# cvjena/semantic-embeddings

Hardware: AMD Instinct MI355X
Metric: retrieval_Mpairs_per_sec (higher is better)
Workload: dtype f32

## Files before the change

### semantic-embeddings_amd/csrc/rank_rows.hip

```cpp
#include "se_common.h"
#include <stdlib.h>
#include <atomic>
#include <type_traits>

namespace se {

constexpr int RK_THREADS = 512;
constexpr int RK_WAVES = RK_THREADS / WAVE;
constexpr int RK_ITEMS = 16;
constexpr int RK_TILE = RK_THREADS * RK_ITEMS;
constexpr int RK_WCHUNK = RK_TILE / RK_WAVES;
constexpr int RK_NB = 256;

struct RankLds {
    uint32_t gbase[4][RK_NB];
    uint32_t wcnt[RK_WAVES][RK_NB];
    uint32_t tile_start[RK_NB];
    uint32_t wave_tot[RK_WAVES];
    uint32_t tkeys[RK_TILE];
    uint32_t tidx[RK_TILE];
};

__device__ __forceinline__ uint32_t wave_excl_scan(uint32_t v, uint32_t &total)
{
    const uint32_t incl = wave_incl_scan(v);
    total = (uint32_t)__builtin_amdgcn_readlane((int)incl, 63);
    return incl - v;
}

template <bool IDX64>
__global__ __launch_bounds__(RK_THREADS) void rank_rows_kernel(const float *__restrict__ pdist, int64_t ldp,
                                                               int64_t Q, int N, void *rank, int64_t ldr,
                                                               uint32_t *ws, int64_t n_pad)
{
    extern __shared__ __attribute__((aligned(16))) unsigned char rk_raw[];
    RankLds &L = *reinterpret_cast<RankLds *>(rk_raw);
    const int tid = threadIdx.x, lane = tid & 63, wave = tid >> 6;
    const uint64_t lt_mask = (lane == 0) ? 0ull : (~0ull >> (64 - lane));

    uint32_t *kA = ws + (int64_t)blockIdx.x * 4 * n_pad;
    uint32_t *iA = kA + n_pad, *kB = iA + n_pad, *iB = kB + n_pad;
    const int ntiles = (N + RK_TILE - 1) / RK_TILE;

    for (int64_t row = blockIdx.x; row < Q; row += gridDim.x) {
        const float *drow = pdist + row * ldp;

        wg_barrier();
        for (int i = tid; i < 4 * RK_NB; i += RK_THREADS) (&L.gbase[0][0])[i] = 0;
        wg_barrier();
        for (int i = tid; i < N; i += RK_THREADS) {
            const uint32_t key = canon_key(drow[i]);
            atomicAdd(&L.gbase[0][key & 0xFF], 1u);
            atomicAdd(&L.gbase[1][(key >> 8) & 0xFF], 1u);
            atomicAdd(&L.gbase[2][(key >> 16) & 0xFF], 1u);
            atomicAdd(&L.gbase[3][key >> 24], 1u);
        }
        wg_barrier();
        if (wave < 4) {
            uint32_t c[4], s = 0;
#pragma unroll
            for (int j = 0; j < 4; j++) { c[j] = L.gbase[wave][lane * 4 + j]; s += c[j]; }
            uint32_t tot;
            uint32_t run = wave_excl_scan(s, tot);
#pragma unroll
            for (int j = 0; j < 4; j++) { L.gbase[wave][lane * 4 + j] = run; run += c[j]; }
        }
        wg_barrier();

#pragma unroll 1
        for (int p = 0; p < 4; p++) {
            const int shift = p * 8;
            const uint32_t *sk = (p & 1) ? kA : kB;
            const uint32_t *si = (p & 1) ? iA : iB;
            uint32_t *dk = (p & 1) ? kB : kA;
            uint32_t *di = (p & 1) ? iB : iA;
            const bool last = (p == 3);
#pragma unroll 1
            for (int t = 0; t < ntiles; t++) {
                const int tbase = t * RK_TILE;
                const int tcount = (N - tbase < RK_TILE) ? (N - tbase) : RK_TILE;
                const int wbeg = wave * RK_WCHUNK;

                uint32_t key[RK_ITEMS], idx[RK_ITEMS];
                if (p == 0) {
#pragma unroll
                    for (int s = 0; s < RK_ITEMS; s++) {
                        const int li = wbeg + s * WAVE + lane;
                        const int gi = tbase + li;
                        const float f = drow[gi < N ? gi : N - 1];
                        key[s] = (li < tcount) ? canon_key(f) : 0xFFFFFFFFu;
                        idx[s] = (uint32_t)gi;
                    }
                } else {
#pragma unroll
                    for (int s = 0; s < RK_ITEMS; s++) {
                        const int li = wbeg + s * WAVE + lane;
                        const int gi = tbase + li;
                        const int gc = gi < N ? gi : N - 1;
                        const uint32_t k = sk[gc], i2 = si[gc];
                        key[s] = (li < tcount) ? k : 0xFFFFFFFFu;
                        idx[s] = i2;
                    }
                }
#pragma unroll
                for (int j = 0; j < RK_NB / WAVE; j++) L.wcnt[wave][j * WAVE + lane] = 0;
#pragma unroll
                for (int s = 0; s < RK_ITEMS; s++) {
                    const int li = wbeg + s * WAVE + lane;
                    if (li < tcount) atomicAdd(&L.wcnt[wave][(key[s] >> shift) & 0xFF], 1u);
                }
                wg_barrier();
                uint32_t my_total = 0;
                if (tid < RK_NB) {
                    uint32_t run = 0;
#pragma unroll
                    for (int w = 0; w < RK_WAVES; w++) {
                        const uint32_t c = L.wcnt[w][tid];
                        L.wcnt[w][tid] = run;
                        run += c;
                    }
                    my_total = run;
                    uint32_t wtot;
                    const uint32_t ex = wave_excl_scan(my_total, wtot);
                    if (lane == 63) L.wave_tot[wave] = wtot;
                    L.tile_start[tid] = ex;
                }
                wg_barrier();
                if (tid < RK_NB) {
                    uint32_t add = 0;
                    for (int w = 0; w < wave; w++) add += L.wave_tot[w];
                    const uint32_t st = L.tile_start[tid] + add;
                    L.tile_start[tid] = st;
#pragma unroll
                    for (int w = 0; w < RK_WAVES; w++) L.wcnt[w][tid] += st;
                }
                wg_barrier();

                volatile uint32_t *cur = L.wcnt[wave];
#pragma unroll
                for (int s = 0; s < RK_ITEMS; s++) {
                    const int li = wbeg + s * WAVE + lane;
                    const bool valid = li < tcount;
                    const uint32_t dgt = (key[s] >> shift) & 0xFF;
                    uint64_t peers = __ballot(valid);
#pragma unroll
                    for (int bb = 0; bb < 8; bb++) {
                        const bool bit = (dgt >> bb) & 1u;
                        const uint64_t m = __ballot(bit && valid);
                        peers &= bit ? m : ~m;
                    }
                    if (valid) {
                        const int rnk = __popcll(peers & lt_mask);
                        const int npeers = __popcll(peers);
                        const uint32_t base = cur[dgt];
                        if (rnk == npeers - 1) cur[dgt] = base + (uint32_t)npeers;
                        L.tkeys[base + rnk] = key[s];
                        L.tidx[base + rnk] = idx[s];
                    }
                }
                wg_barrier();

#pragma unroll
                for (int j = 0; j < RK_ITEMS; j++) {
                    const int i = j * RK_THREADS + tid;
                    if (i < tcount) {
                        const uint32_t k = L.tkeys[i];
                        const uint32_t id = L.tidx[i];
                        const uint32_t d = (k >> shift) & 0xFF;
                        const uint32_t gpos = L.gbase[p][d] + ((uint32_t)i - L.tile_start[d]);
                        if (last) {
                            if (IDX64) ((int64_t *)rank)[row * ldr + gpos] = (int64_t)id;
                            else ((int32_t *)rank)[row * ldr + gpos] = (int32_t)id;
                        } else {
                            dk[gpos] = k;
                            di[gpos] = id;
                        }
                    }
                }
                wg_barrier();
                if (tid < RK_NB) L.gbase[p][tid] += my_total;
            }
        }
    }
}


constexpr int RR_THREADS = 512;
constexpr int RR_WAVES = RR_THREADS / WAVE;
constexpr int RR_SCAN_THREADS = 512;
constexpr int RR_SCAN_WAVES = RR_SCAN_THREADS / WAVE;
static_assert((53248 + RR_THREADS - 1) / RR_THREADS <= 104, "rows of up to 53,248 columns: 104 keys per thread");
constexpr int RR_G = 8;
constexpr int RR_MAX_N = 53248;

__device__ __forceinline__ void differ_mask(uint32_t d, uint32_t &lo, uint32_t &hi)
{
    lo = 0;
    hi = 0;
#pragma unroll
    for (int bb = 0; bb < 8; bb += 2) {
        uint32_t s0 = (uint32_t)__builtin_amdgcn_sbfe((int)d, bb, 1);
        uint32_t s1 = (uint32_t)__builtin_amdgcn_sbfe((int)d, bb + 1, 1);
        asm volatile("" : "+v"(s0), "+v"(s1));
        const uint64_t m0 = __ballot(s0 != 0), m1 = __ballot(s1 != 0);
        lo = __builtin_amdgcn_bitop3_b32(lo, (uint32_t)m0, s0, 0xF6);
        hi = __builtin_amdgcn_bitop3_b32(hi, (uint32_t)(m0 >> 32), s0, 0xF6);
        lo = __builtin_amdgcn_bitop3_b32(lo, (uint32_t)m1, s1, 0xF6);
        hi = __builtin_amdgcn_bitop3_b32(hi, (uint32_t)(m1 >> 32), s1, 0xF6);
    }
}

constexpr uint32_t RR_KEY_NAN = 0xFF900000u;
__device__ __forceinline__ uint32_t rr_pad_key(uint32_t lane) { return 0xFFA00000u + ((lane % 6u) << 20) + (lane << 11) + lane; }
__device__ __forceinline__ uint32_t rr_key(uint32_t u, bool pad, uint32_t pad_key)
{
    const uint32_t sx = (uint32_t)((int32_t)u >> 31);
    uint32_t k = __builtin_amdgcn_bitop3_b32(u, sx, 0x80000000u, 0x1E);
    k -= sx;
    const float f = __uint_as_float(u);
    k = (f != f) ? RR_KEY_NAN : k;
    return pad ? pad_key : k;
}

__device__ __forceinline__ int32_t rr_clamp_i32(int32_t x, int32_t lo, int32_t hi) { return min(max(x, lo), hi); }

template <typename T>
__device__ __forceinline__ void opaque(T &x) { asm volatile("" : "+v"(x)); }

__device__ __forceinline__ uint32_t lds_off(const void *p) { return (uint32_t)(uintptr_t)p; }
__device__ __forceinline__ void lds_wait() { asm volatile("s_waitcnt lgkmcnt(0)" ::: "memory"); }
__device__ __forceinline__ void lds_st16_lo(uint32_t addr, uint32_t v) { asm volatile("ds_write_b16 %0, %1" ::"v"(addr), "v"(v) : "memory"); }
__device__ __forceinline__ void lds_st16_hi(uint32_t addr, uint32_t v) { asm volatile("ds_write_b16_d16_hi %0, %1" ::"v"(addr), "v"(v) : "memory"); }
__device__ __forceinline__ uint32_t rr_dst_mad(uint32_t ir, uint32_t xb)
{
    uint32_t a;
    asm("v_mad_u32_u16 %0, %1, 2, %2" : "=v"(a) : "v"(ir), "s"(xb));
    return a;
}
template <int OFF>
__device__ __forceinline__ void lds_ld16(uint32_t &dst, uint32_t addr) { asm volatile("ds_read_u16 %0, %1 offset:%2" : "=v"(dst) : "v"(addr), "n"(OFF) : "memory"); }
template <int K>
__device__ __forceinline__ void lds_wait_le(uint32_t &landed) { asm volatile("s_waitcnt lgkmcnt(%1)" : "+v"(landed) : "n"(K) : "memory"); }

constexpr int RR_RING = 12;
template <int ITEMS, bool HI, int I = 0>
struct RRRead {
    static __device__ __forceinline__ void run(uint32_t (&a)[ITEMS], uint32_t (&t)[RR_RING], uint32_t addr)
    {
        constexpr int D = RR_RING - 1;
        if constexpr (I < ITEMS) lds_ld16<I * WAVE * 2>(t[I % RR_RING], addr);
        if constexpr (I >= D) {
            constexpr int J = I - D;
            constexpr int newest = (I < ITEMS ? I : ITEMS - 1);
            lds_wait_le<newest - J>(t[J % RR_RING]);
            a[J] = __builtin_amdgcn_perm(t[J % RR_RING], a[J], HI ? 0x05040100u : 0x03020504u);
        }
        if constexpr (I + 1 < ITEMS + D) RRRead<ITEMS, HI, I + 1>::run(a, t, addr);
    }
};

template <int ITEMS, int V, int S0, int I = 0>
struct RRRankFinish {
    static __device__ __forceinline__ void run(uint32_t (&ir)[ITEMS], uint32_t (&key)[ITEMS], uint32_t (&rnk)[V], uint32_t (&base)[V])
    {
        lds_wait_le<2 * (V - 1 - I) + 1>(base[I]);
        ir[S0 + I] = (ir[S0 + I] & 0xFFFF0000u) | (base[I] + rnk[I]);
        opaque(ir[S0 + I]);
        opaque(key[S0 + I]);
        if constexpr (I + 1 < V) RRRankFinish<ITEMS, V, S0, I + 1>::run(ir, key, rnk, base);
    }
};

template <int ITEMS, int S0 = 0>
struct RRRank {
    static __device__ __forceinline__ void run(uint32_t (&ir)[ITEMS], uint32_t (&key)[ITEMS], int shift, int lane, uint32_t cb)
    {
        constexpr int V = (ITEMS - S0 < RR_G) ? (ITEMS - S0) : RR_G;
        static_assert(2 * V - 1 <= 15, "lgkmcnt counts to 15");
        uint32_t rnk[V], base[V];
#pragma unroll
        for (int g = 0; g < V; g++) {
            const uint32_t d = (key[S0 + g] >> shift) & 0xFFu;
            uint32_t dlo, dhi;
            differ_mask(d, dlo, dhi);
            rnk[g] = (uint32_t)lane - wave_prefix_count(dlo, dhi);
            const uint32_t ca = cb + (d << 2);
            asm volatile("ds_read_b32 %0, %1" : "=v"(base[g]) : "v"(ca) : "memory");
            if (rnk[g] == 0) {
                const uint32_t np = 64u - (uint32_t)(__popc(dlo) + __popc(dhi));
                asm volatile("ds_add_u32 %0, %1" ::"v"(ca), "v"(np) : "memory");
            }
        }
        RRRankFinish<ITEMS, V, S0>::run(ir, key, rnk, base);
        __builtin_amdgcn_sched_barrier(0);
        if constexpr (S0 + V < ITEMS) RRRank<ITEMS, S0 + V>::run(ir, key, shift, lane, cb);
    }
};

typedef int rr_i32x4 __attribute__((ext_vector_type(4)));
typedef long long rr_i64x2 __attribute__((ext_vector_type(2)));
constexpr int RR_GH = 8;
constexpr int RR_HW_BITS = 11;
constexpr int RR_WIDE_WORDS = 2048;
constexpr uint32_t RR_TWO_SPAN = (1u << 24) - 3u;
constexpr int RR_TWO_OUT = 256;
constexpr int RR_IMG_RUN = 8;
constexpr int RR_IMG_WL = 3072;
constexpr int RR_IMG_MAX_ITEMS = 98;
constexpr uint32_t RR_IMG_NAN_PADHI = 0xFF0u;
constexpr int RR_IMG_SET_WORDS = 2048;
template <int ITEMS, bool PEEL, int S = 0>
struct RRRankHW {
    static __device__ __forceinline__ void run(uint32_t (&ir)[ITEMS], uint32_t (&key)[ITEMS], uint32_t (&r)[RR_GH], uint32_t (&sh)[RR_GH],
                                               uint32_t (&grp)[RR_GH], uint32_t shift, uint32_t hshift, uint32_t wlo, uint32_t whi, uint32_t cb,
                                               int lane, bool peel)
    {
        constexpr int SLOT = S % RR_GH;
        uint32_t ca = 0, inc = 0, shv = 0, g = 0xFFFFFFFFu;
        uint64_t part = ~0ull;
        if constexpr (S < ITEMS) {
            const uint32_t w = __builtin_amdgcn_ubfe(key[S], shift, wlo);
            const uint32_t h = __builtin_amdgcn_ubfe(key[S], hshift, whi);
            ca = cb + (w << 2);
            if constexpr (PEEL) {
                shv = h << 4;
                inc = 1u << shv;
            } else {
                inc = __umul24(h, 0xFFFFu) + 1u;
                shv = __umul24(h, 0x0202u) + 0x07060100u;
            }
            if constexpr (PEEL) {
                if (peel) {
                    const uint32_t d = w | (h << 11);
                    const bool in = (d == (uint32_t)__builtin_amdgcn_readfirstlane((int)d));
                    const uint64_t m = __ballot(in);
                    if (in) g = wave_prefix_count(m);
                    if (lane == 0) inc = (uint32_t)__popcll(m) << shv;
                    part = ~m | 1ull;
                }
            }
        }
        if constexpr (S >= RR_GH) {
            constexpr int J = S - RR_GH;
            constexpr int younger = ((S < ITEMS ? S : ITEMS) - 1) - J;
            lds_wait_le<younger>(r[SLOT]);
            if constexpr (PEEL) {
                const uint32_t lead = (uint32_t)__builtin_amdgcn_readfirstlane((int)r[SLOT]);
                const uint32_t own = (grp[SLOT] != 0xFFFFFFFFu) ? lead : r[SLOT];
                const uint32_t rank = __builtin_amdgcn_ubfe(own, sh[SLOT], 16u) + (grp[SLOT] != 0xFFFFFFFFu ? grp[SLOT] : 0u);
                ir[J] = (ir[J] & 0xFFFF0000u) | rank;
            } else {
                ir[J] = __builtin_amdgcn_perm(ir[J], r[SLOT], sh[SLOT]);
            }
            opaque(ir[J]);
            opaque(key[J]);
        }
        if constexpr (S < ITEMS) {
            sh[SLOT] = shv;
            grp[SLOT] = g;
            if constexpr (PEEL) {
                uint64_t saved;
                r[SLOT] = 0;
                asm volatile("s_and_saveexec_b64 %0, %4\n\tds_add_rtn_u32 %1, %2, %3\n\ts_mov_b64 exec, %0"
                             : "=&s"(saved), "+v"(r[SLOT])
                             : "v"(ca), "v"(inc), "s"(part)
                             : "memory");
            } else {
                asm volatile("ds_add_rtn_u32 %0, %1, %2" : "=v"(r[SLOT]) : "v"(ca), "v"(inc) : "memory");
            }
        }
        __builtin_amdgcn_sched_barrier(0);
        if constexpr (S + 1 < ITEMS + RR_GH) RRRankHW<ITEMS, PEEL, S + 1>::run(ir, key, r, sh, grp, shift, hshift, wlo, whi, cb, lane, peel);
    }
};

template <int ITEMS, bool HWORD, int VAR>
constexpr size_t rr_region0_bytes()
{
    const size_t cnt = (size_t)RR_WAVES * (HWORD ? (size_t)(1 << RR_HW_BITS) / 2 : (size_t)RK_NB) * sizeof(uint32_t);
    const size_t img = (size_t)RR_THREADS * ITEMS + 32 + (size_t)RR_IMG_WL * sizeof(uint32_t);
    return (VAR == 3 && img > cnt) ? img : cnt;
}

struct RankSeg {
    int shift;
    int seg_n;
    uint16_t *planes;
    int64_t plane_elems;
};

template <int ITEMS, bool PROF, bool HWORD, int VAR, bool SEG = false>
__global__ __launch_bounds__(RR_THREADS, RR_THREADS / 256) void rank_rows_reg_kernel(const float *__restrict__ pdist, int64_t ldp, int64_t Q,
                                                                    int N, void *rank, int64_t ldr, int idx64, int vec_ok,
                                                                    unsigned long long *prof, const uint32_t *skew_flag, const RankSeg seg)
{
    static_assert(!SEG || (HWORD && VAR == 0 && !PROF), "segment runs: plain hardware-ordered build only");
    if (skew_flag && *skew_flag != (uint32_t)VAR) return;
    constexpr bool PEEL = VAR == 1;
    extern __shared__ __attribute__((aligned(16))) unsigned char rr_raw[];
    constexpr int BITS = HWORD ? RR_HW_BITS : 8;
    constexpr int NB = 1 << BITS;
    constexpr int NPASS = (32 + BITS - 1) / BITS;
    constexpr int CNT_WORDS = HWORD ? NB / 2 : NB;
    constexpr bool WIDE = HWORD && ((size_t)RR_THREADS * ITEMS * sizeof(uint16_t) >= (size_t)RR_WAVES * RR_WIDE_WORDS * sizeof(uint32_t));
    constexpr bool IMG = WIDE && VAR == 3;
    constexpr bool RAWKEYS = IMG || (WIDE && VAR == 2);
    static_assert(VAR != 3 || (WIDE && ITEMS <= RR_IMG_MAX_ITEMS && !SEG), "image path: long-row instantiations with room for the tag plane");
    uint32_t *wcnt = reinterpret_cast<uint32_t *>(rr_raw);
    uint32_t *wave_tot = reinterpret_cast<uint32_t *>(rr_raw + rr_region0_bytes<ITEMS, HWORD, VAR>());
    uint16_t *xbuf = reinterpret_cast<uint16_t *>(wave_tot + 32);
    [[maybe_unused]] uint8_t *tagb = rr_raw;
    [[maybe_unused]] uint32_t *wlist = reinterpret_cast<uint32_t *>(rr_raw + (size_t)RR_THREADS * ITEMS + 32);
    [[maybe_unused]] uint32_t *ictl = wave_tot + 24;
    const int tid = threadIdx.x, lane = tid & 63, wave = tid >> 6;
    [[maybe_unused]] const int wave_s = __builtin_amdgcn_readfirstlane(wave);
    const int wpos0 = wave * (ITEMS * WAVE) + lane;
    const uint32_t xb = lds_off(xbuf);
    const uint32_t rb = xb + 2u * (uint32_t)wpos0;
#define RR_DST(IR) (xb + (((IR) & 0xFFFFu) << 1))
    auto row_ptr = [&](int64_t v) -> const float * {
        if constexpr (SEG) return pdist + (v >> seg.shift) * ldp + (v & ((1 << seg.shift) - 1)) * (int64_t)seg.seg_n;
        else return pdist + v * ldp;
    };
    auto row_len = [&](int64_t v) -> int {
        if constexpr (SEG) {
            const int rest = N - (int)(v & ((1 << seg.shift) - 1)) * seg.seg_n;
            return rest < seg.seg_n ? rest : seg.seg_n;
        } else return N;
    };
    uint32_t t_acc[12] = {0, 0, 0, 0, 0, 0, 0, 0, 0, 0, 0, 0}, t_last = PROF ? (uint32_t)__builtin_amdgcn_s_memtime() : 0;
#define RR_T(i) if constexpr (PROF) { const uint32_t now = (uint32_t)__builtin_amdgcn_s_memtime(); t_acc[i] += now - t_last; t_last = now; } else { asm volatile("" ::: "memory"); __builtin_amdgcn_sched_barrier(0); }

    uint32_t key[ITEMS], ir[ITEMS];
    __amdgpu_buffer_rsrc_t ld_rsrc;
    uint32_t ld_voff = 0;
    uint32_t ring[RR_RING];
#define RR_LOAD_ONE(DROW, WPOS, S, NN)                                                                               \
    {                                                                                                                 \
        if ((S) % 16 == 0) {                                                                                          \
            if ((S) == 0) {                                                                                           \
                ld_rsrc = __builtin_amdgcn_make_buffer_rsrc(const_cast<float *>(DROW), 0, (NN) * 4, 0x00020000);     \
                ld_voff = (uint32_t)(WPOS) * 4u;                                                                      \
            } else ld_voff += 4096u;                                                                                  \
            opaque(ld_voff);                                                                                          \
        }                                                                                                             \
        key[S] = (uint32_t)__builtin_amdgcn_raw_buffer_load_b32(ld_rsrc, (int)ld_voff + ((S) % 16) * 256, 0, 0);      \
    }
#define RR_CANON(NN)                                                                                                  \
    {                                                                                                                 \
        int wpos_ = wpos0;                                                                                            \
        opaque(wpos_);                                                                                                \
        const uint32_t pk_ = rr_pad_key((uint32_t)wpos_ & 63u);                                                       \
        _Pragma("unroll") for (int s = 0; s < ITEMS; s++) {                                                           \
            const int pos = wpos_ + s * WAVE;                                                                         \
            key[s] = rr_key(key[s], pos >= (NN), pk_ + (ITEMS <= 88 ? (uint32_t)((((s >> 3) & 7) << 17) | ((s & 7) << 6)) : 0u));  \
        }                                                                                                             \
    }
#define RR_PREFETCH_NEXT_ROW() RR_PREFETCH_NEXT_ROW_IF(end >= 32 && more)
#define RR_PREFETCH_NEXT_ROW_IF(COND) \
    if (COND) { \
                const char *nrow = (const char *)row_ptr(row + gridDim.x); \
                const uint32_t row_bytes = (uint32_t)row_len(row + gridDim.x) * 4u; \
                for (uint32_t off = (uint32_t)tid * 128u; off < row_bytes; off += RR_THREADS * 128u) \
                    asm volatile("global_load_dword %0, %1, off" : "=v"(pf_sink) : "v"(nrow + off) : "memory"); \
            }
#define RR_STREAM_PLANE(P, ROW)                                                                                       \
    {                                                                                                                 \
        uint16_t *pl = seg.planes + (P) * seg.plane_elems + (ROW) * (int64_t)(RR_THREADS * ITEMS);                    \
        int j = tid * 8;                                                                                              \
        opaque(j);                                                                                                    \
        _Pragma("unroll 2") for (; j < RR_THREADS * ITEMS; j += RR_THREADS * 8)                                       \
            *reinterpret_cast<uint4 *>(pl + j) = *reinterpret_cast<const uint4 *>(xbuf + j);                          \
    }
    constexpr int RR_PADS = ITEMS < 8 ? ITEMS : 8;
#define RR_PAD_LOOP(NROW, BODY)                                                                                       \
    {                                                                                                                 \
        const int first_pad_ = ((NROW) - wave_s * (ITEMS * WAVE)) >> 6;    \
        if (first_pad_ >= ITEMS - RR_PADS) {                                                                          \
            _Pragma("unroll") for (int s = ITEMS - RR_PADS; s < ITEMS; s++) { BODY }                                  \
        } else {                                                                                                      \
            _Pragma("unroll") for (int s = 0; s < ITEMS; s++) { BODY }                                                \
        }                                                                                                             \
    }
#define RR_IDX_SCATTER_IMG(AFTER_STORE)                                                                               \
    {                                                                                                                 \
        opaque(ir[0]);                                                                                                \
        uint32_t a_ = rr_dst_mad(ir[0], xb);                                                                          \
        _Pragma("unroll") for (int s = 0; s < ITEMS; s++) {                                                           \
            uint32_t an_ = 0;                                                                                         \
            if (s + 1 < ITEMS) { opaque(ir[s + 1]); an_ = rr_dst_mad(ir[s + 1], xb); }                                \
            lds_st16_hi(a_, ir[s]);                                                                        \
            AFTER_STORE                                                                                               \
            a_ = an_;                                                                                                 \
        }                                                                                                             \
    }
    if ((int64_t)blockIdx.x < Q) {
        const float *drow = row_ptr(blockIdx.x);
        const int n0 = row_len(blockIdx.x);
        int wpos = wpos0;
        opaque(wpos);
#pragma unroll
        for (int s = 0; s < ITEMS; s++) RR_LOAD_ONE(drow, wpos, s, n0)
        if constexpr (!RAWKEYS) RR_CANON(n0)
    }
    uint32_t pf_sink = 0;
    [[maybe_unused]] int img_level = 0;
    [[maybe_unused]] bool img_again = false;
    [[maybe_unused]] int img_skip0 = 0, img_pen0 = 0, img_skip1 = 0, img_pen1 = 0;
    for (int64_t row = blockIdx.x; row < Q;) {
        const bool more = row + gridDim.x < Q;
        [[maybe_unused]] const int n_next = row_len(more ? row + gridDim.x : row);
        constexpr bool SKIP_WAVES = HWORD && ITEMS <= 88;
        const bool wave_live = !SKIP_WAVES || wave * (ITEMS * WAVE) < row_len(row);
        constexpr bool LOAD_IN_SCATTER = IMG && !SKIP_WAVES;
        bool two = false;
        [[maybe_unused]] int n_out = 0;
        if constexpr (IMG) {
            const int n_row = row_len(row);
            if (!img_again) {
                if (img_skip1 > 0) { img_level = 2; img_skip1--; }
                else if (img_skip0 > 0) { img_level = 1; img_skip0--; }
                else img_level = 0;
            }
            bool attempt = img_level < 2;
            uint32_t cbits = 0, base = 0;
            if (attempt) {
                uint32_t mb = 0;
#pragma unroll
                for (int s = 0; s + 1 < ITEMS; s += 2) mb = max(max(mb, key[s] & 0x7FFFFFFFu), key[s + 1] & 0x7FFFFFFFu);
                if constexpr (ITEMS & 1) mb = max(mb, key[ITEMS - 1] & 0x7FFFFFFFu);
#pragma unroll
                for (int off = 32; off > 0; off >>= 1) mb = max(mb, (uint32_t)__shfl_xor((int)mb, off, 64));
                if (lane == 0) wave_tot[wave] = mb;
                static_assert(!IMG || (RR_IMG_SET_WORDS == 4 * RR_THREADS && RR_IMG_SET_WORDS == RR_WIDE_WORDS && RR_IMG_SET_WORDS <= RR_IMG_WL), "one uint4 per thread, inside the worklist");
                *reinterpret_cast<uint4 *>(wlist + 4 * tid) = make_uint4(0u, 0u, 0u, 0u);
                wg_barrier();
                if (tid == 0) { ictl[0] = 0; ictl[1] = 0; }
#pragma unroll
                for (int w = 0; w < RR_WAVES; w++) mb = max(mb, wave_tot[w]);
                mb = (uint32_t)__builtin_amdgcn_readfirstlane((int)mb);
                const uint32_t e = (mb >> 23) + ((mb & 0x7FFFFFu) > 0x400000u ? 1u : 0u) - (img_level == 0 ? 1u : 0u);
                two = mb >= 0x0D800000u && mb < 0x7E800000u;
                cbits = (e + 1u) << 23;
                base = e << 23;
            }
            if (two) {
                const float c = __uint_as_float(cbits);
                int wpos_ = wpos0;
                opaque(wpos_);
                const uint32_t pk_ = ((RR_IMG_NAN_PADHI + ((uint32_t)wpos_ & 15u)) << 20) | (((uint32_t)wpos_ & 63u) << 14);
                const uint32_t tb = lds_off(tagb) + (uint32_t)wpos_;
#pragma unroll
                for (int s = 0; s < ITEMS; s++) {
                    const uint32_t t = __float_as_uint(__uint_as_float(key[s]) + c);
                    const uint32_t q = (uint32_t)rr_clamp_i32(__builtin_elementwise_sub_sat((int32_t)t, (int32_t)base), 0, 0xFEFFFF);
                    asm volatile("ds_write_b8 %0, %1 offset:%2" ::"v"(tb), "v"(q), "n"(s * WAVE) : "memory");
                    key[s] = q << 8;
                }
                if (wave_s * (ITEMS * WAVE) + ITEMS * WAVE > n_row) {
                    RR_PAD_LOOP(n_row, key[s] = (wpos_ + s * WAVE >= n_row) ? pk_ : key[s];)
                }
            } else {
                RR_CANON(n_row)
            }
            RR_T(8)
        }
        if constexpr (WIDE && VAR == 2) {
            uint32_t *stat = wave_tot;
            uint2 *outl = reinterpret_cast<uint2 *>(wcnt);
            const int n_row = row_len(row);
            int32_t mxi = 0;
            uint32_t umx = 0;
#pragma unroll
            for (int s = 0; s + 1 < ITEMS; s += 2) {
                mxi = max(max(mxi, rr_clamp_i32((int32_t)key[s], 0, 0x7F800000)), rr_clamp_i32((int32_t)key[s + 1], 0, 0x7F800000));
                umx = max(max(umx, key[s]), key[s + 1]);
            }
            if constexpr (ITEMS & 1) { mxi = max(mxi, rr_clamp_i32((int32_t)key[ITEMS - 1], 0, 0x7F800000)); umx = max(umx, key[ITEMS - 1]); }
            mxi = umx > 0xFF800000u ? 0x7F800000 : mxi;
#pragma unroll
            for (int off = 32; off > 0; off >>= 1) mxi = max(mxi, __shfl_xor(mxi, off, 64));
            if (lane == 0) stat[wave] = (uint32_t)mxi;
            if (tid == 0) stat[2 * RR_WAVES] = 0;
            RR_T(9)
            wg_barrier();
            RR_T(10)
#pragma unroll
            for (int w = 0; w < RR_WAVES; w++) mxi = max(mxi, (int32_t)stat[w]);
            const int32_t kmax = __builtin_amdgcn_readfirstlane(mxi);
            const int32_t lo = kmax > (int32_t)RR_TWO_SPAN ? kmax - (int32_t)RR_TWO_SPAN : 1, lo1 = lo - 1;
            uint32_t below_l = 0;
            {
                int wpos = wpos0;
                opaque(wpos);
#pragma unroll
                for (int s = 0; s < ITEMS; s++) below_l += ((int32_t)key[s] < lo) ? 1u : 0u;
                if (wave_s * (ITEMS * WAVE) + ITEMS * WAVE > n_row) {
                    int32_t lo_b = lo;
                    opaque(lo_b);
                    RR_PAD_LOOP(n_row, below_l -= (wpos + s * WAVE >= n_row && (int32_t)key[s] < lo_b) ? 1u : 0u;)
                }
            }
            uint32_t below_w = below_l;
#pragma unroll
            for (int off = 32; off > 0; off >>= 1) below_w += (uint32_t)__shfl_xor((int)below_w, off, 64);
            if (lane == 0) stat[RR_WAVES + wave] = below_w;
            RR_T(11)
            wg_barrier();
            uint32_t below = 0;
#pragma unroll
            for (int w = 0; w < RR_WAVES; w++) below += stat[RR_WAVES + w];
            two = kmax > 0 && below <= (uint32_t)RR_TWO_OUT;
            n_out = (int)below;
            if (two) {
                int wpos = wpos0;
                opaque(wpos);
                if (below_w != 0) {
                    int32_t lo_c = lo;
                    opaque(lo_c);
#pragma unroll
                    for (int s = 0; s < ITEMS; s++)
                        if ((int32_t)key[s] < lo_c && wpos + s * WAVE < n_row)
                            outl[atomicAdd(&stat[2 * RR_WAVES], 1u)] = make_uint2(rr_key(key[s], false, 0u), (uint32_t)(wpos + s * WAVE));
                }
#pragma unroll
                for (int s = 0; s < ITEMS; s++)
                    key[s] = (uint32_t)rr_clamp_i32(__builtin_elementwise_sub_sat((int32_t)key[s], lo1), 0, 0xFFFFFF) << 8;
                if (wave_s * (ITEMS * WAVE) + ITEMS * WAVE > n_row) {
                    RR_PAD_LOOP(n_row, key[s] = (wpos + s * WAVE >= n_row) ? 0xFFFFFF00u : key[s];)
                }
            } else {
                RR_CANON(n_row)
            }
            RR_T(8)
        }
        __builtin_amdgcn_sched_barrier(0);
        {
            int wpos = wpos0;
            opaque(wpos);
#pragma unroll
            for (int s = 0; s < ITEMS; s++) ir[s] = (uint32_t)(wpos + s * WAVE) << 16;
        }
#pragma unroll 1
        for (int p = 0; p < NPASS; p++) {
            const int shift = two ? 8 + 12 * p : (WIDE ? p * 10 : p * BITS);
            const int end = two ? (p == 1 ? 32 : 20)
                                : (WIDE ? (p == 2 ? 32 : shift + 10) : ((shift + BITS < 32) ? shift + BITS : 32));
            const bool wide = WIDE && (two || p == 2);
            uint32_t *pcnt = wcnt;
            int pcw = CNT_WORDS;
            const bool shared0 = IMG && two && p == 0;
            if (shared0) {
                pcnt = wlist;
                pcw = 0;
            } else if (wide) {
                if (!(RAWKEYS && two && p == 0)) wg_barrier();
                pcnt = reinterpret_cast<uint32_t *>(xbuf);
                pcw = RR_WIDE_WORDS;
            }
            uint32_t *mycnt = pcnt + wave * pcw;
            const uint32_t cb = lds_off(mycnt);
            auto one_set = [&]() -> bool {
                if constexpr (!IMG) return false;
                int z = pcw;
                asm volatile("" : "+s"(z));
                return z == 0;
            };
            if constexpr (IMG) {
                if (!one_set()) {
#pragma unroll
                    for (int j = 0; j < CNT_WORDS / (4 * WAVE); j++) reinterpret_cast<uint4 *>(mycnt)[j * WAVE + lane] = make_uint4(0u, 0u, 0u, 0u);
                    if (wide) {
#pragma unroll
                        for (int j = CNT_WORDS / (4 * WAVE); j < RR_WIDE_WORDS / (4 * WAVE); j++) reinterpret_cast<uint4 *>(mycnt)[j * WAVE + lane] = make_uint4(0u, 0u, 0u, 0u);
                    }
                }
            } else {
#pragma unroll
                for (int j = 0; j < CNT_WORDS / WAVE; j++) mycnt[j * WAVE + lane] = 0;
                if (wide) {
#pragma unroll
                    for (int j = CNT_WORDS / WAVE; j < RR_WIDE_WORDS / WAVE; j++) mycnt[j * WAVE + lane] = 0;
                }
            }
            [[maybe_unused]] const uint32_t wlo = wide ? 11u : 10u, whi = (uint32_t)(end - shift) - wlo, hshift = (uint32_t)(shift + (int)wlo) & 31u;
            if constexpr (HWORD) {
                if (wave_live) {
                    uint32_t hr[RR_GH], hs[RR_GH], hg[RR_GH];
                    RRRankHW<ITEMS, PEEL>::run(ir, key, hr, hs, hg, (uint32_t)shift, hshift, wlo, whi, cb, lane, end >= 32 && !two);
                }
            }
            else RRRank<ITEMS>::run(ir, key, shift, lane, cb);
            lds_wait();
            RR_T(1)
            wg_barrier();
            if constexpr (!HWORD) {
            uint32_t ex = 0;
            if (tid < RK_NB) {
                uint32_t run = 0;
#pragma unroll
                for (int w = 0; w < RR_WAVES; w++) run += wcnt[w * RK_NB + tid];
                uint32_t wtot;
                ex = wave_excl_scan(run, wtot);
                if (lane == 63) wave_tot[wave] = wtot;
            }
            wg_barrier();
            if (tid < RK_NB) {
                for (int w = 0; w < wave; w++) ex += wave_tot[w];
#pragma unroll
                for (int w = 0; w < RR_WAVES; w++) {
                    const uint32_t c = wcnt[w * RK_NB + tid];
                    wcnt[w * RK_NB + tid] = ex;
                    ex += c;
                }
            }
            } else {
                const bool scanner = tid < RR_SCAN_THREADS;
                const int st = scanner ? tid : 0;
                uint32_t T0 = 0, T1 = 0, U0 = 0, U1 = 0;
#pragma unroll
                for (int w = 0; w < RR_WAVES; w++) {
                    if (w == 1 && one_set()) break;
                    const uint2 v = *reinterpret_cast<const uint2 *>(pcnt + w * pcw + 2 * st);
                    T0 += v.x; T1 += v.y;
                }
                if (wide) {
                    __builtin_amdgcn_sched_barrier(0);
#pragma unroll
                    for (int w = 0; w < RR_WAVES; w++) {
                        if (w == 1 && one_set()) break;
                        const uint2 v = *reinterpret_cast<const uint2 *>(pcnt + w * pcw + CNT_WORDS + 2 * st);
                        U0 += v.x; U1 += v.y;
                    }
                    __builtin_amdgcn_sched_barrier(0);
                }
                uint32_t wtot, wtot2 = 0, ex2 = 0;
                uint32_t ex = wave_excl_scan(T0 + T1, wtot);
                if (wide) ex2 = wave_excl_scan(U0 + U1, wtot2);
                if (scanner && lane == 63) { wave_tot[wave] = wtot; wave_tot[RR_SCAN_WAVES + wave] = wtot2; }
                wg_barrier();
                uint32_t all = 0, all2 = 0;
#pragma unroll
                for (int w = 0; w < RR_SCAN_WAVES; w++) {
                    const uint32_t wt = wave_tot[w], wt2 = wave_tot[RR_SCAN_WAVES + w];
                    all += wt; all2 += wt2;
                    ex += (w < wave) ? wt : 0u;
                    ex2 += (w < wave) ? wt2 : 0u;
                }
                ex2 += all;
                const uint32_t hi = (all + all2) << 16;
                ex += hi; ex2 += hi;
                if (scanner) {
                uint32_t s0 = ex, s1 = ex + T0;
#pragma unroll
                for (int w = 0; w < RR_WAVES; w++) {
                    if (w == 1 && one_set()) break;
                    uint2 *wp = reinterpret_cast<uint2 *>(pcnt + w * pcw + 2 * tid);
                    const uint2 v = *wp;
                    *wp = make_uint2(s0, s1);
                    s0 += v.x; s1 += v.y;
                }
                if (wide) {
                    __builtin_amdgcn_sched_barrier(0);
                    s0 = ex2; s1 = ex2 + U0;
#pragma unroll
                    for (int w = 0; w < RR_WAVES; w++) {
                        if (w == 1 && one_set()) break;
                        uint2 *wp = reinterpret_cast<uint2 *>(pcnt + w * pcw + CNT_WORDS + 2 * tid);
                        const uint2 v = *wp;
                        *wp = make_uint2(s0, s1);
                        s0 += v.x; s1 += v.y;
                    }
                }
                }
            }
            wg_barrier();
            RR_T(2)
            if (!(IMG && two)) { RR_PREFETCH_NEXT_ROW() }
            if (wave_live) {
#pragma unroll
            for (int s0 = 0; s0 < ITEMS; s0 += 8) {
                uint32_t first[8];
#pragma unroll
                for (int g = 0; g < 8; g++)
                    if (s0 + g < ITEMS) {
                        if constexpr (HWORD) first[g] = reinterpret_cast<const uint16_t *>(mycnt)[(__builtin_amdgcn_ubfe(key[s0 + g], (uint32_t)shift, wlo) << 1) | __builtin_amdgcn_ubfe(key[s0 + g], hshift, whi)];
                        else first[g] = mycnt[(key[s0 + g] >> shift) & 0xFFu];
                    }
#pragma unroll
                for (int g = 0; g < 8; g++)
                    if (s0 + g < ITEMS) {
                        ir[s0 + g] += first[g];
                        opaque(ir[s0 + g]);
                    }
                __builtin_amdgcn_sched_barrier(0);
            }
            }
            if (wide && !one_set()) wg_barrier();
            RR_T(3)
            if constexpr (LOAD_IN_SCATTER) {
                if (end >= 32) break;
            }
            if (wave_live) {
                if constexpr (LOAD_IN_SCATTER) {
                    RR_IDX_SCATTER_IMG()
                } else {
#pragma unroll
                    for (int s = 0; s < ITEMS; s++) { opaque(ir[s]); lds_st16_hi(RR_DST(ir[s]), ir[s]); }
                }
            }
            lds_wait();
            wg_barrier();
            RR_T(4)
            const bool last = end >= 32;
            if (last) {
                if constexpr (!SEG) break;
                else {
                    RR_STREAM_PLANE(0, row)
                    wg_barrier();
                }
            } else {
                if (wave_live) RRRead<ITEMS, true>::run(ir, ring, rb);
                lds_wait();
                wg_barrier();
            }
            RR_T(5)
            if (wave_live) {
#pragma unroll
                for (int s = 0; s < ITEMS; s++) { opaque(ir[s]); lds_st16_hi(RR_DST(ir[s]), key[s]); }
            }
            lds_wait();
            wg_barrier();
            if (SEG && last) {
                RR_STREAM_PLANE(1, row)
            } else {
                if (wave_live) RRRead<ITEMS, true>::run(key, ring, rb);
                lds_wait();
            }
            if (end < 16 || SEG) {
                wg_barrier();
                if (wave_live) {
#pragma unroll
                    for (int s = 0; s < ITEMS; s++) { opaque(ir[s]); lds_st16_lo(RR_DST(ir[s]), key[s]); }
                }
                lds_wait();
                wg_barrier();
                if (SEG && last) break;
                if (wave_live) RRRead<ITEMS, false>::run(key, ring, rb);
                lds_wait();
            }
            RR_T(6)
        }
#undef RR_DST
        if constexpr (WIDE && VAR == 2) {
            if (two && n_out > 1) {
                const uint2 *outl = reinterpret_cast<const uint2 *>(wcnt);
                if (tid < n_out) {
                    const uint2 me = outl[tid];
                    int r = 0;
                    for (int j = 0; j < n_out; j++) {
                        const uint2 o = outl[j];
                        r += (o.x < me.x || (o.x == me.x && o.y < me.y)) ? 1 : 0;
                    }
                    xbuf[r] = (uint16_t)me.y;
                }
                wg_barrier();
            }
        }
        [[maybe_unused]] bool img_fail = false;
        if constexpr (IMG) {
            const float *drow = row_ptr(more ? row + gridDim.x : row);
            int wpos = wpos0;
            opaque(wpos);
            if constexpr (LOAD_IN_SCATTER) {
                RR_IDX_SCATTER_IMG(RR_LOAD_ONE(drow, wpos, s, n_next))
                lds_wait();
                wg_barrier();
                RR_T(4)
            } else {
#pragma unroll
                for (int s = 0; s < ITEMS; s++) RR_LOAD_ONE(drow, wpos, s, n_next)
            }
        }
        if constexpr (IMG) {
            if (two) {
                int n_row = row_len(row);
                int tsc = wave_s * WAVE + (int)wave_prefix_count(~0u, ~0u);
                opaque(n_row);
                opaque(tsc);
                const float *drow_cur = row_ptr(row);
                constexpr int NS = RR_THREADS * ITEMS;
                constexpr int NG = (NS / 8 + RR_THREADS - 1) / RR_THREADS;
                uint32_t S[NG];
                uint32_t nstart = 0;
                uint4 xg[NG];
                uint32_t nxg[NG];
#pragma unroll
                for (int g = 0; g < NG; g++) {
                    const int b0 = (tsc + RR_THREADS * g) * 8;
                    const int bs = b0 < NS ? b0 : 0;
                    xg[g] = *reinterpret_cast<const uint4 *>(xbuf + bs);
                    nxg[g] = xbuf[(tsc & 63) == 63 ? (bs + 8 < NS ? bs + 8 : bs) : 0];
                }
                constexpr int TD = 1;
                uint32_t t[TD + 1][9];
                auto tag_reads = [&](int g, uint32_t (&tt)[9]) {
                    const uint32_t xi[4] = {xg[g].x, xg[g].y, xg[g].z, xg[g].w};
#pragma unroll
                    for (int j = 0; j < 4; j++) {
                        tt[2 * j] = tagb[xi[j] & 0xFFFFu];
                        tt[2 * j + 1] = tagb[xi[j] >> 16];
                    }
                    tt[8] = tagb[nxg[g]];
                };
#pragma unroll
                for (int g = 0; g < TD && g < NG; g++) tag_reads(g, t[g % (TD + 1)]);
#pragma unroll
                for (int g = 0; g < NG; g++) {
                    if (g + TD < NG) tag_reads(g + TD, t[(g + TD) % (TD + 1)]);
                    const uint32_t (&tc)[9] = t[g % (TD + 1)];
                    const bool live = (tsc + RR_THREADS * g) * 8 < n_row - 1;
                    const uint32_t A = tc[0] | (tc[1] << 8) | (tc[2] << 16) | (tc[3] << 24), B = tc[4] | (tc[5] << 8) | (tc[6] << 16) | (tc[7] << 24);
                    const uint32_t t8 = (uint32_t)__builtin_amdgcn_update_dpp((int)tc[8], (int)tc[0], 0x130, 0xF, 0xF, false);
                    const uint32_t zA = A ^ __builtin_amdgcn_alignbyte(B, A, 1), zB = B ^ __builtin_amdgcn_alignbyte(t8, B, 1);
                    const uint32_t uA = (zA & 0x7F7F7F7Fu) + 0x7F7F7F7Fu, uB = (zB & 0x7F7F7F7Fu) + 0x7F7F7F7Fu;
                    const uint32_t eA = __builtin_amdgcn_bitop3_b32(uA, zA, 0x80808080u, 0x02), eB = __builtin_amdgcn_bitop3_b32(uB, zB, 0x80808080u, 0x02);
                    S[g] = live ? ((eA >> 7) | (eB >> 3)) : 0u;
                    nstart += (uint32_t)__popc(S[g]);
                }
                uint32_t slot = 0;
                {
                    const uint32_t ca = lds_off(&ictl[0]);
                    asm volatile("ds_add_rtn_u32 %0, %1, %2\n\ts_waitcnt lgkmcnt(0)" : "=v"(slot) : "v"(ca), "v"(nstart) : "memory");
                }
#pragma unroll
                for (int g = 0; g < NG; g++) {
                    uint32_t st = S[g];
                    const int b0 = (tsc + RR_THREADS * g) * 8;
                    while (st) {
                        const int bit = __builtin_ctz(st);
                        st &= st - 1u;
                        const int pos = b0 + (bit & 4) + (bit >> 3);
                        if (slot < (uint32_t)RR_IMG_WL) wlist[slot] = pos < n_row - 1 ? (uint32_t)pos : 0xFFFFFFFFu;
                        slot++;
                    }
                }
                if constexpr (PROF) { RR_T(9) }
                wg_barrier();
                const uint32_t nwork = ictl[0];
                img_fail = nwork > (uint32_t)RR_IMG_WL;
                RR_T(11)
                if (!img_fail) {
                    constexpr int GB = 2;
#pragma unroll 1
                    for (uint32_t e0 = 0; e0 < nwork; e0 += RR_THREADS * GB) {
                        uint32_t pp[GB], im[GB], ia[GB], ib[GB], ic[GB], id[GB], tm[GB], t0[GB], t2[GB], t3[GB], ka[GB], kb[GB], kc[GB];
#pragma unroll
                        for (int k = 0; k < GB; k++) {
                            const uint32_t e = e0 + (uint32_t)(k * RR_THREADS + tsc);
                            pp[k] = e < nwork ? wlist[e] : 0xFFFFFFFFu;
                        }
#pragma unroll
                        for (int k = 0; k < GB; k++) {
                            const uint32_t p = pp[k] != 0xFFFFFFFFu ? pp[k] : 0u;
                            im[k] = xbuf[p ? p - 1u : 0u]; ia[k] = xbuf[p]; ib[k] = xbuf[p + 1];
                            ic[k] = xbuf[p + 2 < (uint32_t)NS ? p + 2 : p]; id[k] = xbuf[p + 3 < (uint32_t)NS ? p + 3 : p];
                        }
#pragma unroll
                        for (int k = 0; k < GB; k++) { tm[k] = tagb[im[k]]; t0[k] = tagb[ia[k]]; t2[k] = tagb[ic[k]]; t3[k] = tagb[id[k]]; }
#pragma unroll
                        for (int k = 0; k < GB; k++) {
                            const bool mine = pp[k] != 0xFFFFFFFFu && !(pp[k] != 0u && tm[k] == t0[k]);
                            const bool three = mine && (int)pp[k] + 2 < n_row && t2[k] == t0[k];
                            ka[k] = kb[k] = kc[k] = 0u;
                            if (mine) {
                                ka[k] = __float_as_uint(drow_cur[ia[k]]);
                                kb[k] = __float_as_uint(drow_cur[ib[k]]);
                            }
                            if (three) kc[k] = __float_as_uint(drow_cur[ic[k]]);
                        }
                        uint32_t rare = 0;
#pragma unroll
                        for (int k = 0; k < GB; k++) {
                            if (pp[k] == 0xFFFFFFFFu) continue;
                            const uint32_t p = pp[k];
                            if (p != 0u && tm[k] == t0[k]) continue;
                            const bool three = (int)p + 2 < n_row && t2[k] == t0[k];
                            const bool more4 = three && (int)p + 3 < n_row && t3[k] == t0[k];
                            const uint64_t ca = ((uint64_t)rr_key(ka[k], false, 0u) << 32) | ia[k], cb = ((uint64_t)rr_key(kb[k], false, 0u) << 32) | ib[k],
                                           cc = ((uint64_t)rr_key(kc[k], false, 0u) << 32) | ic[k];
                            if (!three) {
                                if (ca > cb) { xbuf[p] = (uint16_t)ib[k]; xbuf[p + 1] = (uint16_t)ia[k]; }
                            } else if (!more4) {
                                const uint32_t ab = ca < cb, ac = ca < cc, bc = cb < cc;
                                const uint32_t ra = 2u - ab - ac, rb = ab + 1u - bc, rc = ac + bc;
                                if (ra != 0u || rb != 1u) {
                                    xbuf[p + ra] = (uint16_t)ia[k]; xbuf[p + rb] = (uint16_t)ib[k]; xbuf[p + rc] = (uint16_t)ic[k];
                                }
                            } else rare |= 1u << k;
                        }
                        static_assert(GB == 2, "the entry is picked by one select");
#pragma unroll 1
                        for (uint32_t k = 0; k < (uint32_t)GB; k++) {
                            if (!((rare >> k) & 1u)) continue;
                            const uint32_t p = k ? pp[1] : pp[0], tg = k ? t0[1] : t0[0];
                            int len = 4;
                            while (len <= RR_IMG_RUN && (int)p + len < n_row && tagb[xbuf[p + len]] == tg) len++;
                            if (len > RR_IMG_RUN) { ictl[1] = 1u; continue; }
                            uint32_t idx[RR_IMG_RUN];
                            uint64_t kk[RR_IMG_RUN];
#pragma unroll
                            for (int j = 0; j < RR_IMG_RUN; j++) idx[j] = xbuf[p + (uint32_t)(j < len ? j : 0)];
#pragma unroll
                            for (int j = 0; j < RR_IMG_RUN; j++) kk[j] = ((uint64_t)rr_key(__float_as_uint(drow_cur[idx[j]]), false, 0u) << 32) | idx[j];
#pragma unroll
                            for (int j = 0; j < RR_IMG_RUN; j++) {
                                uint32_t r = 0;
#pragma unroll
                                for (int i = 0; i < RR_IMG_RUN; i++)
                                    if (i != j) r += (i < len && kk[i] < kk[j]) ? 1u : 0u;
                                if (j < len) xbuf[p + r] = (uint16_t)idx[j];
                            }
                        }
                    }
                    wg_barrier();
                    img_fail = ictl[1] != 0u;
                }
                RR_T(10)
            }
        }
        if (!IMG || img_fail) {
            const float *drow = row_ptr((IMG && img_fail) ? row : (more ? row + gridDim.x : row));
            int wpos = wpos0;
            opaque(wpos);
#pragma unroll
            for (int s = 0; s < ITEMS; s++) RR_LOAD_ONE(drow, wpos, s, n_next)
        }
        if constexpr (IMG) {
#pragma unroll
            for (int s = 0; s < ITEMS; s++) opaque(key[s]);
            asm volatile("s_waitcnt vmcnt(0)" : "+v"(pf_sink) : : "memory");
        }
        int wt = tid;
        opaque(wt);
        const bool write_out = !IMG || !img_fail;
        if constexpr (SEG) {
            RR_STREAM_PLANE(2, row)
        } else if (!write_out) {
        } else if (idx64 == 2) {
            uint16_t *o = (uint16_t *)rank + row * ldr;
            _Pragma("unroll 2") for (int j = wt * 8; j < N; j += RR_THREADS * 8) {
                if (vec_ok && j + 7 < N) {
                    const rr_i32x4 v = *reinterpret_cast<const rr_i32x4 *>(xbuf + j);
                    __builtin_nontemporal_store(v, reinterpret_cast<rr_i32x4 *>(o + j));
                } else {
                    for (int e = 0; e < 8 && j + e < N; e++) o[j + e] = xbuf[j + e];
                }
            }
        } else if (idx64) {
            int64_t *o = (int64_t *)rank + row * ldr;
            uint2 nv = *reinterpret_cast<const uint2 *>(xbuf + (wt * 4 < N ? wt * 4 : 0));
            _Pragma("unroll 1") for (int j = wt * 4; j < N; j += RR_THREADS * 4) {
                const uint2 v = nv;
                const int jn = j + RR_THREADS * 4;
                nv = *reinterpret_cast<const uint2 *>(xbuf + (jn < N ? jn : 0));
                const int64_t e0 = v.x & 0xFFFFu, e1 = v.x >> 16, e2 = v.y & 0xFFFFu, e3 = v.y >> 16;
                if (vec_ok && j + 3 < N) {
                    __builtin_nontemporal_store((rr_i64x2){e0, e1}, reinterpret_cast<rr_i64x2 *>(o + j));
                    __builtin_nontemporal_store((rr_i64x2){e2, e3}, reinterpret_cast<rr_i64x2 *>(o + j + 2));
                } else {
                    o[j] = e0;
                    if (j + 1 < N) o[j + 1] = e1;
                    if (j + 2 < N) o[j + 2] = e2;
                    if (j + 3 < N) o[j + 3] = e3;
                }
            }
        } else {
            int32_t *o = (int32_t *)rank + row * ldr;
            constexpr int RR_WO = 4;
            _Pragma("unroll 1") for (int j0 = wt * 4; j0 < N; j0 += RR_THREADS * 4 * RR_WO) {
                uint2 v[RR_WO];
#pragma unroll
                for (int u = 0; u < RR_WO; u++) {
                    const int j = j0 + u * RR_THREADS * 4;
                    v[u] = *reinterpret_cast<const uint2 *>(xbuf + (j < N ? j : 0));
                }
#pragma unroll
                for (int u = 0; u < RR_WO; u++) {
                    const int j = j0 + u * RR_THREADS * 4;
                    if (j >= N) break;
                    const int e0 = v[u].x & 0xFFFFu, e1 = v[u].x >> 16, e2 = v[u].y & 0xFFFFu, e3 = v[u].y >> 16;
                    if (vec_ok && j + 3 < N) {
                        __builtin_nontemporal_store((rr_i32x4){e0, e1, e2, e3}, reinterpret_cast<rr_i32x4 *>(o + j));
                    } else {
                        o[j] = e0;
                        if (j + 1 < N) o[j + 1] = e1;
                        if (j + 2 < N) o[j + 2] = e2;
                        if (j + 3 < N) o[j + 3] = e3;
                    }
                }
            }
        }
        RR_T(7)
        if constexpr (!RAWKEYS) RR_CANON(n_next)
        if constexpr (PROF) {
            _Pragma("unroll") for (int s = 0; s < ITEMS; s++) opaque(key[s]);
        }
        if constexpr (!IMG)
            asm volatile("s_waitcnt vmcnt(0)" : "+v"(pf_sink) : : "memory");
        RR_T(0)
        if constexpr (IMG) {
            if (img_fail) {
                if (img_level == 0) { img_pen0 = img_pen0 ? (img_pen0 < 16 ? 2 * img_pen0 : 32) : 1; img_skip0 = img_pen0; }
                else { img_pen1 = img_pen1 ? (img_pen1 < 16 ? 2 * img_pen1 : 32) : 1; img_skip1 = img_pen1; }
                img_level++;
                img_again = true;
            } else {
                if (two) { if (img_level == 0) img_pen0 = 0; else img_pen1 = 0; }
                img_again = false;
                row += gridDim.x;
            }
        } else row += gridDim.x;
    }
    if (PROF && tid == 0)
    {
        for (int i = 0; i < 12; i++) atomicAdd(&prof[i], (unsigned long long)t_acc[i]);
    }
#undef RR_T
}

}

using namespace se;

static size_t rank_idx_bytes(int idx) { return idx == 2 ? 2 : (idx ? 8 : 4); }

static int rank_grid(int64_t q)
{
    const int64_t g = 512;
    return (int)(q < g ? q : g);
}

static int64_t rank_npad(int64_t n) { return (n + 63) / 64 * 64; }

static bool rank_use_tiled(int64_t n)
{
    static const bool force = tuning_env("SE_RANK_TILED") != nullptr;
    return force || n > RR_MAX_N;
}

__global__ __launch_bounds__(256) void rank_skew_detect_kernel(const float *__restrict__ pdist, int64_t ldp, int64_t Q, int N,
// ... 781 lines not shown
```

Before: 236,800.

## Read back scattered 16-bit keys with transposed 64-bit LDS loads

```diff
diff --git a/semantic-embeddings_amd/csrc/rank_rows.hip b/semantic-embeddings_amd/csrc/rank_rows.hip
--- a/semantic-embeddings_amd/csrc/rank_rows.hip
+++ b/semantic-embeddings_amd/csrc/rank_rows.hip
@@ -239,25 +239,47 @@
 }
 template <int OFF>
 __device__ __forceinline__ void lds_ld16(uint32_t &dst, uint32_t addr) { asm volatile("ds_read_u16 %0, %1 offset:%2" : "=v"(dst) : "v"(addr), "n"(OFF) : "memory"); }
-template <int K>
-__device__ __forceinline__ void lds_wait_le(uint32_t &landed) { asm volatile("s_waitcnt lgkmcnt(%1)" : "+v"(landed) : "n"(K) : "memory"); }
+template <int OFF>
+__device__ __forceinline__ void lds_ld16x4_tr(uint64_t &dst, uint32_t addr) { asm volatile("ds_read_b64_tr_b16 %0, %1 offset:%2" : "=v"(dst) : "v"(addr), "n"(OFF) : "memory"); }
+template <int K, typename T>
+__device__ __forceinline__ void lds_wait_le(T &landed) { asm volatile("s_waitcnt lgkmcnt(%1)" : "+v"(landed) : "n"(K) : "memory"); }
 
 constexpr int RR_RING = 12;
+__host__ __device__ constexpr uint32_t rr_tr_lane_off(uint32_t lane) { return 128u * ((lane >> 2) & 3u) + 32u * (lane >> 4) + 8u * (lane & 3u); }
 template <int ITEMS, bool HI, int I = 0>
 struct RRRead {
-    static __device__ __forceinline__ void run(uint32_t (&a)[ITEMS], uint32_t (&t)[RR_RING], uint32_t addr)
+    static constexpr int NT = ITEMS / 4, OPS = NT + ITEMS % 4, D = RR_RING / 2 - 1;
+    static constexpr uint32_t SEL_LO16 = HI ? 0x05040100u : 0x03020504u;
+    static constexpr uint32_t SEL_HI16 = HI ? 0x07060100u : 0x03020706u;
+    static __device__ __forceinline__ void run(uint32_t (&a)[ITEMS], uint64_t (&t)[RR_RING / 2], uint32_t (&u)[4], uint32_t rt, uint32_t rb)
     {
-        constexpr int D = RR_RING - 1;
-        if constexpr (I < ITEMS) lds_ld16<I * WAVE * 2>(t[I % RR_RING], addr);
+        if constexpr (I < NT) lds_ld16x4_tr<I * 4 * WAVE * 2>(t[I % (RR_RING / 2)], rt);
+        else if constexpr (I < OPS) lds_ld16<(3 * NT + I) * WAVE * 2>(u[I - NT], rb);
         if constexpr (I >= D) {
             constexpr int J = I - D;
-            constexpr int newest = (I < ITEMS ? I : ITEMS - 1);
-            lds_wait_le<newest - J>(t[J % RR_RING]);
-            a[J] = __builtin_amdgcn_perm(t[J % RR_RING], a[J], HI ? 0x05040100u : 0x03020504u);
-        }
-        if constexpr (I + 1 < ITEMS + D) RRRead<ITEMS, HI, I + 1>::run(a, t, addr);
+            constexpr int newest = (I < OPS ? I : OPS - 1);
+            if constexpr (J < NT) {
+                uint64_t &v = t[J % (RR_RING / 2)];
+                lds_wait_le<newest - J>(v);
+                const uint32_t lo = (uint32_t)v, hi = (uint32_t)(v >> 32);
+                a[4 * J + 0] = __builtin_amdgcn_perm(lo, a[4 * J + 0], SEL_LO16);
+                a[4 * J + 1] = __builtin_amdgcn_perm(lo, a[4 * J + 1], SEL_HI16);
+                a[4 * J + 2] = __builtin_amdgcn_perm(hi, a[4 * J + 2], SEL_LO16);
+                a[4 * J + 3] = __builtin_amdgcn_perm(hi, a[4 * J + 3], SEL_HI16);
+            } else {
+                lds_wait_le<newest - J>(u[J - NT]);
+                a[3 * NT + J] = __builtin_amdgcn_perm(u[J - NT], a[3 * NT + J], SEL_LO16);
+            }
+        }
+        if constexpr (I + 1 < OPS + D) RRRead<ITEMS, HI, I + 1>::run(a, t, u, rt, rb);
     }
 };
+template <int ITEMS, bool HI>
+__device__ __forceinline__ void rr_read_back(uint32_t (&a)[ITEMS], uint64_t (&ring)[RR_RING / 2], uint32_t rt, uint32_t rb)
+{
+    uint32_t u[4];
+    RRRead<ITEMS, HI>::run(a, ring, u, rt, rb);
+}
 
 template <int ITEMS, int V, int S0, int I = 0>
 struct RRRankFinish {
@@ -389,8 +411,10 @@
     int64_t plane_elems;
 };
 
+template <int ITEMS, bool HWORD, bool SEG>
+constexpr int rr_code_align() { return (HWORD && !SEG && ITEMS >= 88) ? 65536 : 256; }
 template <int ITEMS, bool PROF, bool HWORD, int VAR, bool SEG = false>
-__global__ __launch_bounds__(RR_THREADS, RR_THREADS / 256) void rank_rows_reg_kernel(const float *__restrict__ pdist, int64_t ldp, int64_t Q,
+__global__ __launch_bounds__(RR_THREADS, RR_THREADS / 256) __attribute__((aligned(rr_code_align<ITEMS, HWORD, SEG>()))) void rank_rows_reg_kernel(const float *__restrict__ pdist, int64_t ldp, int64_t Q,
                                                                     int N, void *rank, int64_t ldr, int idx64, int vec_ok,
                                                                     unsigned long long *prof, const uint32_t *skew_flag, const RankSeg seg)
 {
@@ -417,6 +441,8 @@
     const int wpos0 = wave * (ITEMS * WAVE) + lane;
     const uint32_t xb = lds_off(xbuf);
     const uint32_t rb = xb + 2u * (uint32_t)wpos0;
+    static_assert(rr_region0_bytes<ITEMS, HWORD, VAR>() % 16 == 0 && (ITEMS * WAVE * sizeof(uint16_t)) % 8 == 0, "transposed reads need 8-byte aligned addresses");
+    [[maybe_unused]] const uint32_t rt = xb + 2u * (uint32_t)(wave * (ITEMS * WAVE)) + rr_tr_lane_off((uint32_t)lane);
 #define RR_DST(IR) (xb + (((IR) & 0xFFFFu) << 1))
     auto row_ptr = [&](int64_t v) -> const float * {
         if constexpr (SEG) return pdist + (v >> seg.shift) * ldp + (v & ((1 << seg.shift) - 1)) * (int64_t)seg.seg_n;
@@ -434,7 +460,7 @@
     uint32_t key[ITEMS], ir[ITEMS];
     __amdgpu_buffer_rsrc_t ld_rsrc;
     uint32_t ld_voff = 0;
-    uint32_t ring[RR_RING];
+    uint64_t ring[RR_RING / 2];
 #define RR_LOAD_ONE(DROW, WPOS, S, NN)                                                                               \
     {                                                                                                                 \
         if ((S) % 16 == 0) {                                                                                          \
@@ -820,7 +846,7 @@
                     wg_barrier();
                 }
             } else {
-                if (wave_live) RRRead<ITEMS, true>::run(ir, ring, rb);
+                if (wave_live) rr_read_back<ITEMS, true>(ir, ring, rt, rb);
                 lds_wait();
                 wg_barrier();
             }
@@ -834,7 +860,7 @@
             if (SEG && last) {
                 RR_STREAM_PLANE(1, row)
             } else {
-                if (wave_live) RRRead<ITEMS, true>::run(key, ring, rb);
+                if (wave_live) rr_read_back<ITEMS, true>(key, ring, rt, rb);
                 lds_wait();
             }
             if (end < 16 || SEG) {
@@ -846,7 +872,7 @@
                 lds_wait();
                 wg_barrier();
                 if (SEG && last) break;
-                if (wave_live) RRRead<ITEMS, false>::run(key, ring, rb);
+                if (wave_live) rr_read_back<ITEMS, false>(key, ring, rt, rb);
                 lds_wait();
             }
             RR_T(6)
```

Measured after the change: 243,600, median of 6. 2.9% higher.
